# JonasGeiping/breaching

Hardware: NVIDIA H100
Metric: reconstruction iters/sec (ResNet-18 224x224, invertinggradients) (higher is better)
Workload: dtype tf32

## Files before the change

### breaching_b200/csrc/engine.cu

```cuda
#include <math.h>
#include <stdlib.h>
#include <string.h>

#include <limits>
#include <string>
#include <vector>

#include "../../include/breaching_b200.h"
#include "common.cuh"
#include "igemm.cuh"
#include "layers.cuh"
#include "tokens.cuh"
#include "objective.cuh"
#include "augment.cuh"

namespace bre {
void set_pdl(bool on);
static thread_local std::string g_last_error;
void set_error(const std::string& msg) { g_last_error = msg; }
static int g_pdl = -1;
bool use_pdl() {
  if (g_pdl < 0) {
    const char* e = getenv("BRE_PDL");
    g_pdl = e ? (atoi(e) != 0) : 1;
// ... 312 lines not shown
      a.x_sN = g.Ci; a.x_sP = g.Ci; a.x_sC = 1;
    } else {
      g.N = ti.N; g.H = ti.H; g.W = ti.W; g.Ci = ti.C; g.Ho = to.H; g.Wo = to.W; g.Co = to.C;
      g.R = op.R; g.S = op.S; g.stride = op.stride; g.pad = op.pad;
      if (op.tin == 0) { a.x_sN = (long long)ti.C * ti.H * ti.W; a.x_sP = 1; a.x_sC = ti.H * ti.W; }
      else { a.x_sN = (long long)ti.H * ti.W * ti.C; a.x_sP = ti.C; a.x_sC = 1; }
    }
    a.nsrc = 1;
    a.ws = ws; a.counters = gemm_counters; a.ws_tiles = ws_tiles; a.splits = 0;
    a.force_fp32 = is_precise(op_index(op)) ? 1 : 0;
    return a;
  }
  int gemm(const GemmArgs& a) { return gemm_on(a, stream); }
  bool weight_prefetch = [] { const char* e = getenv("BRE_TC_WPREFETCH"); return e ? atoi(e) != 0 : true; }();
  bool v_settled = false;
  bool inside(const float* p, const float* base, long long n) const { return base != nullptr && p >= base && p < base + n; }
  unsigned static_weights(const GemmArgs& a) const {
    if (!weight_prefetch || ms_steps > 0 || a.mode == GEMM_WGRAD) return 0u;
    unsigned mask = 0;
    for (int s = 0; s < a.nsrc; ++s) {
      const float* p = a.wgt[s];
      const bool model = inside(p, W, P_pad) || inside(p, Wt, P_pad) || (Wcol != nullptr && p == Wcol);
      const bool direction = v_settled && (inside(p, V, P_pad) || inside(p, Vt, P_pad));
      if (model || direction) mask |= 1u << s;
    }
    return mask;
  }
  int gemm_on(const GemmArgs& a, cudaStream_t st) {
    if (linear_tall_supported(a)) return launch_linear_tall(a, st);
    if (linear_small_preferred(a)) return launch_linear_small(a, st);
    if (gemm_backend == 1 && !a.force_fp32 && igemm_tc_supported(a)) {
      GemmArgs b = a;
      b.wgt_static = static_weights(a);
      return launch_igemm_tc(b, st);
    }
    return launch_igemm_simt(a, st);
  }

  bool fuses_with_next(size_t i, const GemmArgs& a) const {
    if (!fuse_bnact || gemm_backend != 1 || i + 1 >= ops.size()) return false;
    const bre_op_desc& nx = ops[i + 1];
    return nx.kind == BRE_OP_BNACT && nx.tin == ops[i].tout && !nx.bn_train && igemm_tc_supported(a);
  }
  std::vector<unsigned char> op_flags;
  void clear_op_flags(unsigned char bits) {
    op_flags.resize(ops.size(), 0);
    for (unsigned char& f : op_flags) f &= (unsigned char)~bits;
  }
  int consumers_of(int tensor) const {
    int n = 0;
    for (const bre_op_desc& o : ops) n += (o.tin == tensor) + (o.res == tensor);
    return n;
  }

  BnTrainArgs bn_train_args(const bre_op_desc& op) {
    const bre_tensor_desc& to = td(op.tout);
    const BnBuf& b = bn[op.bn_buffer];
    BnTrainArgs a;
    memset(&a, 0, sizeof(a));
    a.P = (long long)to.N * to.H * to.W; a.C = to.C; a.relu = op.relu != 0;
    a.in = t[op.tin].val; a.out = t[op.tout].val;
    a.inv = b.inv; a.nrm = b.nrm; a.scale = b.scale;
    a.v_gamma = Vp(op.gamma); a.v_beta = Vp(op.beta);
    a.sum_du = Gp(op.beta); a.sum_duxh = Gp(op.gamma);
    a.m1 = b.di_cm; a.m2 = b.di_cv; a.b1 = b.tb1; a.b2 = b.tb2;
    a.dout = t[op.tout].d; a.tdout = t[op.tout].td; a.xd = t[op.tin].tval;
// ... 1657 lines not shown
```

### breaching_b200/csrc/igemm.cuh

```cuda
#pragma once
#include "common.cuh"

namespace bre {

enum GemmMode { GEMM_FPROP = 0, GEMM_DGRAD = 1, GEMM_WGRAD = 2 };

struct ConvGeom {
  int N, H, W, Ci;
  int Ho, Wo, Co;
  int R, S, stride, pad;
};

struct GemmEpilogue {
  int kind;
  int has_bn, relu;
  int round_out;
  float* out2;
  const float* res;
  const float* scale;
  const float* shift;
  const float* inv;
  const float* nrm;
  const float* v_gamma;
  const float* v_beta;
  const float* pre;
  const float* post;
};

struct GemmArgs {
  int mode;
  GemmEpilogue epi;
  ConvGeom g;
  int nsrc;
  const float* act[2];
  const float* wgt[2];
  long long x_sN;
  int x_sP, x_sC;
  float* out;
  const float* bias;
  int accumulate;
  float* ws;
  int* counters;
  int ws_tiles;
  int splits;
  int force_fp32;
  unsigned wgt_static;
};

constexpr int IG_BM = 64, IG_BN = 64, IG_BK = 16, IG_THREADS = 256;

int launch_igemm_simt(const GemmArgs& a, cudaStream_t stream);
bool linear_small_supported(const GemmArgs& a);
int launch_linear_small(const GemmArgs& a, cudaStream_t stream);
bool linear_small_preferred(const GemmArgs& a);
bool linear_tall_supported(const GemmArgs& a);
int launch_linear_tall(const GemmArgs& a, cudaStream_t stream);
int launch_igemm_tc(const GemmArgs& a, cudaStream_t stream);
bool igemm_tc_supported(const GemmArgs& a);

inline void gemm_dims(const GemmArgs& a, int& M, int& Nc, int& K) {
  const ConvGeom& g = a.g;
  if (a.mode == GEMM_FPROP) { M = g.N * g.Ho * g.Wo; Nc = g.Co; K = g.R * g.S * g.Ci; }
  else if (a.mode == GEMM_DGRAD) { M = g.N * g.H * g.W; Nc = g.Ci; K = g.R * g.S * g.Co; }
  else { M = g.Co; Nc = g.R * g.S * g.Ci; K = g.N * g.Ho * g.Wo; }
}

}
```

### breaching_b200/csrc/igemm_tc.cu

```cuda
#include <stdlib.h>
#include <string.h>

#include <array>
#include <map>
#include <mutex>
#include <type_traits>

#include <cuda.h>

#include "igemm.cuh"

namespace bre {

namespace {

constexpr int TC_BM = 128;
constexpr int TC_BK = 32;
constexpr int TC_STAGES = 4;
constexpr int TC_MAX_STAGES = 8;
constexpr int TC_THREADS = 128;
constexpr int TC_BLOCK = 2 * TC_THREADS;

struct TcDims {
  int M, Nc, K;
// ... 138 lines not shown
               ::"r"(dst), "l"(reinterpret_cast<uint64_t>(tm)), "r"(smem_u32(bar)), "r"(c0), "r"(c1), "r"(c2) : "memory");
}

template <int NV>
__device__ __forceinline__ void fused_bnact(const GemmEpilogue& e, long long row, int n, float (&v)[NV]) {
  const long long o = row + n;
#pragma unroll
  for (int j = 0; j < NV; ++j) {
    float u = v[j];
    if (e.kind == 1) {
      if (e.has_bn) u = fmaf(u, __ldg(e.scale + n + j), __ldg(e.shift + n + j));
      if (e.res != nullptr) u += e.res[o + j];
      u = e.relu ? fmaxf(u, 0.f) : u;
      v[j] = e.round_out ? tf32_rna(u) : u;
    } else {
      if (e.has_bn) {
        const float xhat = fmaf(e.pre[o + j], __ldg(e.inv + n + j), __ldg(e.nrm + n + j));
        u = fmaf(__ldg(e.scale + n + j), u, fmaf(__ldg(e.v_gamma + n + j), xhat, __ldg(e.v_beta + n + j)));
      }
      if (e.res != nullptr) u += e.res[o + j];
      if (e.relu && !(e.post[o + j] > 0.f)) u = 0.f;
      v[j] = e.round_out ? tf32_rna(u) : u;
    }
  }
}

#ifdef BRE_TC_TRACE
__device__ long long g_tc_trace[16];
#define TC_MARK(i, cond) do { if ((cond) && blockIdx.x == 0 && blockIdx.y == 0 && blockIdx.z == 0) g_tc_trace[i] = clock64(); } while (0)
#else
#define TC_MARK(i, cond) do { } while (0)
#endif

template <int MODE, int BN, bool TMA, bool CLS = false>
__global__ void __launch_bounds__(TC_BLOCK) igemm_tc_kernel(GemmArgs a, TcDims d, int proxy_fence,
                                                            const __grid_constant__ std::conditional_t<CLS, TcMapsCls, TcMaps> maps, ClsPlan plan) {
  static_assert(!CLS || (MODE == GEMM_DGRAD && TMA), "per-class gathers: strided dgrad with the TMA producer only");
  constexpr uint32_t A_BYTES = TC_BM * TC_BK * 4, B_BYTES = BN * TC_BK * 4;
  extern __shared__ __align__(1024) uint8_t smem[];
  uint8_t* sA = smem;
  const int nst = 1 << d.stage_shift, stage_mask = nst - 1;
  uint8_t* sB = smem + nst * A_BYTES;
  __shared__ __align__(8) uint64_t bar_full[TC_MAX_STAGES];
  __shared__ __align__(8) uint64_t bar_empty[TC_MAX_STAGES];

  TC_MARK(0, threadIdx.x == 0);
  pdl_launch_dependents();
  const ConvGeom g = a.g;
  const int tid = threadIdx.x, warp = tid >> 5, lane = tid & 31;
  const int ptid = tid & (TC_THREADS - 1);
  const bool consumer = warp < TC_THREADS / 32;
  const int n0 = blockIdx.y * BN, z = blockIdx.z;
  int m0 = blockIdx.x * TC_BM;
  int kb_begin = z * d.kblocks_per_split;
  int kb_end = min(d.total_kblocks, kb_begin + d.kblocks_per_split);
  const int HoWo = g.Ho * g.Wo, HW = g.H * g.W;
  int cls = 0, cHc = 0, cWc = 0, cTy = 0, cTx = 0, cls_kps = 0, Mrows = d.M;
  if (CLS) {
#pragma unroll
    for (int c = 1; c < TC_MAXCLS; ++c)
      if (c < plan.ncls && (int)blockIdx.x >= plan.tile0[c]) cls = c;
    m0 = ((int)blockIdx.x - plan.tile0[cls]) * TC_BM;
    cHc = plan.Hc[cls]; cWc = plan.Wc[cls]; cTy = plan.Ty[cls]; cTx = plan.Tx[cls];
    Mrows = g.N * cHc * cWc;
    cls_kps = cTy * cTx * (g.Co / TC_BK);
    const int total = cls_kps * a.nsrc, per = (total + (int)gridDim.z - 1) / (int)gridDim.z;
    kb_begin = z * per;
    kb_end = min(total, kb_begin + per);
  }

  if (tid == 0) {
#pragma unroll
    for (int s = 0; s < TC_MAX_STAGES; ++s) { mbar_init(&bar_full[s], TMA ? 1 : TC_THREADS); mbar_init(&bar_empty[s], TC_THREADS / 32); }
    fence_barrier_init();
  }
  __syncthreads();
  TC_MARK(1, threadIdx.x == 0);

  constexpr bool a_mn = MODE == GEMM_WGRAD;
  constexpr bool b_mn = MODE != GEMM_FPROP;

  constexpr int A_VEC = TC_BM * TC_BK / 4 / TC_THREADS;
  constexpr int B_VEC = BN * TC_BK / 4 / TC_THREADS;
  const int gcol = ptid & 7, grow = (ptid >> 3) & 15;
  int a_off[A_VEC];
  unsigned long long a_taps[A_VEC];
  int a_yx[A_VEC];
  if (!TMA && !consumer && (MODE == GEMM_FPROP || MODE == GEMM_DGRAD)) {
#pragma unroll
    for (int j = 0; j < A_VEC; ++j) {
      const int m = m0 + grow + 16 * j;
      a_off[j] = 0; a_taps[j] = 0ull; a_yx[j] = 0;
      if (m < d.M) {
        if (MODE == GEMM_FPROP) {
          const int img = m / HoWo, rem = m - img * HoWo;
          const int p = rem / g.Wo, q = rem - p * g.Wo;
          const int y0 = p * g.stride - g.pad, x0 = q * g.stride - g.pad;
          a_off[j] = (int)(img * a.x_sN) + (y0 * g.W + x0) * a.x_sP + gcol * 4;
          for (int r = 0; r < g.R; ++r)
            for (int s2 = 0; s2 < g.S; ++s2)
              if (y0 + r >= 0 && y0 + r < g.H && x0 + s2 >= 0 && x0 + s2 < g.W) a_taps[j] |= 1ull << (r * g.S + s2);
        } else {
          const int img = m / HW, rem = m - img * HW;
          const int y = rem / g.W, x = rem - y * g.W;
          const int yb = y + g.pad, xb = x + g.pad;
          const int py = yb / g.stride, qx = xb / g.stride;
          const int ey = yb - py * g.stride, ex = xb - qx * g.stride;
          a_off[j] = ((img * g.Ho + py) * g.Wo + qx) * g.Co + gcol * 4;
          a_yx[j] = (ey << 16) | ex;
          for (int r = ey, pp = py; r < g.R; r += g.stride, --pp)
            for (int s2 = ex, qq = qx; s2 < g.S; s2 += g.stride, --qq)
              if (pp >= 0 && pp < g.Ho && qq >= 0 && qq < g.Wo) a_taps[j] |= 1ull << (r * g.S + s2);
        }
      }
    }
// ... 63 lines not shown
      return;
    }
    if (MODE == GEMM_WGRAD) {
      if (st.c0 >= d.kblocks_per_src * TC_BK) { st.c0 = 0; ++st.src; st.img = st.p = st.q = 0; }
      else {
        st.q += TC_BK;
        while (st.q >= g.Wo) { st.q -= g.Wo; if (++st.p == g.Ho) { st.p = 0; ++st.img; } }
      }
    } else if (st.c0 >= kch) {
      st.c0 = 0; ++st.rs;
      if (++st.s == g.S) { st.s = 0; if (++st.r == g.R) { st.r = 0; st.rs = 0; ++st.src; } }
    }
  };
  int wg_c[BN / 32], wg_r[BN / 32], wg_s[BN / 32];
  if (TMA && MODE == GEMM_WGRAD) {
#pragma unroll
    for (int h = 0; h < BN / 32; ++h) {
      const int n = n0 + 32 * h;
      const int rs = n / g.Ci;
      wg_c[h] = n - rs * g.Ci; wg_r[h] = rs / g.S; wg_s[h] = rs - wg_r[h] * g.S;
    }
  }
  auto issue_wgt_tma = [&](int stage, const KbState& st) {
    uint64_t* bar = &bar_full[stage];
    const uint32_t pb = smem_u32(sB) + stage * B_BYTES;
    if (MODE == GEMM_FPROP) {
      tma_tile2d(pb, &maps.wgt[st.src], bar, st.rs * g.Ci + st.c0, n0);
    } else if (MODE == GEMM_DGRAD) {
#pragma unroll
      for (int h = 0; h < BN / 32; ++h) tma_tile3d(pb + h * 4096, &maps.wgt[st.src], bar, n0 + 32 * h, st.rs, st.c0);
    } else {
      const uint32_t pa = smem_u32(sA) + stage * A_BYTES;
#pragma unroll
      for (int h = 0; h < TC_BM / 32; ++h) tma_tile2d(pa + h * 4096, &maps.wgt[st.src], bar, m0 + 32 * h, st.c0);
    }
  };
  auto issue_act_tma = [&](int stage, const KbState& st) {
    uint64_t* bar = &bar_full[stage];
    const uint32_t pa = smem_u32(sA) + stage * A_BYTES, pb = smem_u32(sB) + stage * B_BYTES;
    if (MODE == GEMM_FPROP) {
      tma_im2col(pa, &maps.act[st.src], bar, st.c0, base_w, base_h, base_n, st.s, st.r);
    } else if (MODE == GEMM_DGRAD) {
      if (CLS) tma_im2col(pa, &maps.act[2 * cls + st.src], bar, st.c0, base_w, base_h, base_n, cTx - 1 - st.s, cTy - 1 - st.r);
      else tma_im2col(pa, &maps.act[st.src], bar, st.c0, base_w, base_h, base_n, g.S - 1 - st.s, g.R - 1 - st.r);
    } else {
#pragma unroll
      for (int h = 0; h < BN / 32; ++h)
        tma_im2col(pb + h * 4096, &maps.act[st.src], bar, wg_c[h], st.q * g.stride - g.pad, st.p * g.stride - g.pad, st.img, wg_s[h], wg_r[h]);
    }
  };

  if (TMA && tid == 0 && (proxy_fence & 2)) {
    for (int sidx = 0; sidx < a.nsrc; ++sidx) {
      asm volatile("prefetch.tensormap [%0];" ::"l"(reinterpret_cast<uint64_t>(&maps.act[(CLS ? 2 * cls : 0) + sidx])) : "memory");
      asm volatile("prefetch.tensormap [%0];" ::"l"(reinterpret_cast<uint64_t>(&maps.wgt[sidx])) : "memory");
    }
  }
  const int nprod = (proxy_fence >> 2) & 7;
  const int pw = warp - TC_THREADS / 32;
  const bool producer = TMA && !consumer && lane == 0 && pw < nprod && pw < nkb;
  KbState pst;
  memset(&pst, 0, sizeof(pst));
  uint32_t pre_wgt = 0;
  if (producer) {
    pst = kb_init(kb_begin + pw);
    if (MODE != GEMM_WGRAD && a.wgt_static != 0) {
      KbState st = pst;
// ... 70 lines not shown
        }
      }
      {
        const int n4 = ptid & 15, kk = ptid >> 4;
        const int n = n0 + n4 * 4;
        const int rs = n / g.Ci, c = n - rs * g.Ci;
        const int r = rs / g.S, s = rs - r * g.S;
#pragma unroll
        for (int j = 0; j < B_VEC; ++j) {
          const int k = kk + 8 * j;
          const int pix = kbase + k;
          bool ok = pix < d.K;
          const float* gb = act;
          if (ok) {
            const int img = pix / HoWo, rem = pix - img * HoWo;
            const int p = rem / g.Wo, q = rem - p * g.Wo;
            const int h = p * g.stride - g.pad + r, w = q * g.stride - g.pad + s;
            ok = h >= 0 && h < g.H && w >= 0 && w < g.W;
            if (ok) gb = act + img * a.x_sN + (long long)(h * g.W + w) * a.x_sP + c;
          }
          cp_async16(pb + off_mn128(4 * n4, k), gb, ok ? 16u : 0u);
        }
      }
    }
    it_c0 += TC_BK;
    if (MODE == GEMM_WGRAD) {
      if (it_c0 >= d.kblocks_per_src * TC_BK) { it_c0 = 0; ++it_src; }
    } else if (it_c0 >= kch) {
      it_c0 = 0;
      if (++it_rs == g.R * g.S) { it_rs = 0; ++it_src; }
    }
  };

  float acc[2][BN / 2];
#pragma unroll
  for (int h = 0; h < 2; ++h)
#pragma unroll
    for (int i = 0; i < BN / 2; ++i) acc[h][i] = 0.f;
  const int gq = lane >> 2, tq = lane & 3;
  if (consumer) {
    for (int i = 0; i < nkb; ++i) {
      const int stage = i & stage_mask;
      mbar_wait(&bar_full[stage], (uint32_t)((i >> d.stage_shift) & 1));
      TC_MARK(4, i == 0 && tid == 0);
      if constexpr (MODE == GEMM_FPROP) {
        if (!TMA || (proxy_fence & 1)) fence_proxy_async();
        const uint32_t sa = smem_u32(sA) + stage * A_BYTES, sb = smem_u32(sB) + stage * B_BYTES;
        wgmma_fence();
#pragma unroll
        for (int j = 0; j < TC_BK / 8; ++j) {
          const uint64_t db = wgmma_desc_k128(sb + 32 * j);
          wgmma_tf32<BN>(acc[0], wgmma_desc_k128(sa + 32 * j), db);
          wgmma_tf32<BN>(acc[1], wgmma_desc_k128(sa + 64 * 128 + 32 * j), db);
        }
        wgmma_commit();
        wgmma_wait<1>();
        fence_regs(acc[0]);
        fence_regs(acc[1]);
        __syncwarp();
        if (i > 0 && lane == 0) mbar_arrive(&bar_empty[(i - 1) & stage_mask]);
      } else {
        const uint8_t* pa = sA + stage * A_BYTES;
        const uint8_t* pb = sB + stage * B_BYTES;
#pragma unroll
        for (int j = 0; j < TC_BK / 8; ++j) {
          const int k0 = 8 * j + tq;
          uint32_t af[2][4];
#pragma unroll
          for (int h = 0; h < 2; ++h) {
            const int r = 64 * h + 16 * warp + gq;
            af[h][0] = ld_op<a_mn>(pa, r, k0);
            af[h][1] = ld_op<a_mn>(pa, r + 8, k0);
            af[h][2] = ld_op<a_mn>(pa, r, k0 + 4);
            af[h][3] = ld_op<a_mn>(pa, r + 8, k0 + 4);
          }
#pragma unroll
          for (int jn = 0; jn < BN / 8; ++jn) {
            const uint32_t b0 = ld_op<b_mn>(pb, 8 * jn + gq, k0), b1 = ld_op<b_mn>(pb, 8 * jn + gq, k0 + 4);
            mma_tf32(&acc[0][4 * jn], af[0], b0, b1);
            mma_tf32(&acc[1][4 * jn], af[1], b0, b1);
          }
        }
        __syncwarp();
        if (lane == 0) mbar_arrive(&bar_empty[stage]);
      }
    }
    if constexpr (MODE == GEMM_FPROP) {
      wgmma_wait<0>();
      fence_regs(acc[0]);
      fence_regs(acc[1]);
    }
    TC_MARK(5, tid == 0);
  } else {
    if (TMA) {
      if (producer) {
        KbState st = pst;
        for (int i = pw; i < nkb; i += nprod) {
          const int stage = i & stage_mask;
          if (i >= nst) mbar_wait(&bar_empty[stage], (uint32_t)(((i >> d.stage_shift) - 1) & 1));
          if (i >= nst || !((pre_wgt >> i) & 1u)) {
            mbar_expect_tx(&bar_full[stage], A_BYTES + B_BYTES);
            issue_wgt_tma(stage, st);
          }
          issue_act_tma(stage, st);
          TC_MARK(3, i == (nkb < nst ? nkb : nst) - 1);
          for (int u = 0; u < nprod; ++u) kb_advance(st);
        }
      }
      __syncwarp();
    } else {
      for (int i = 0; i < nkb; ++i) {
        const int stage = i & stage_mask;
        if (i >= nst) mbar_wait(&bar_empty[stage], (uint32_t)(((i >> d.stage_shift) - 1) & 1));
        issue_block(stage);
        cp_async_arrive(&bar_full[stage]);
      }
      cp_async_wait<0>();
    }
  }

  const int splits = gridDim.z;
  auto out_row = [&](int mm, long long& row, int& cs) {
    if (CLS) {
      const int per = cHc * cWc;
      const int img = mm / per, rem = mm - img * per;
      const int iy = rem / cWc, ix = rem - iy * cWc;
      row = img * a.x_sN + (long long)((plan.y0[cls] + plan.stride * iy) * g.W + plan.x0[cls] + plan.stride * ix) * a.x_sP;
      cs = a.x_sC;
    } else if (MODE == GEMM_DGRAD) {
      const int img = mm / HW;
      row = img * a.x_sN + (long long)(mm - img * HW) * a.x_sP;
      cs = a.x_sC;
    } else {
      row = (long long)mm * d.Nc;
      cs = 1;
    }
  };
  if (consumer && splits == 1) {
#pragma unroll
    for (int h = 0; h < 2; ++h) {
#pragma unroll
      for (int hr = 0; hr < 2; ++hr) {
        const int mm = m0 + 64 * h + 16 * warp + gq + 8 * hr;
        if (mm >= Mrows) continue;
        long long row;
        int cs;
        out_row(mm, row, cs);
#pragma unroll
        for (int jn = 0; jn < BN / 8; ++jn) {
          const int n = n0 + 8 * jn + 2 * tq;
          float v[2] = {acc[h][4 * jn + 2 * hr], acc[h][4 * jn + 2 * hr + 1]};
          if (MODE == GEMM_FPROP && a.bias != nullptr) {
            v[0] += __ldg(a.bias + n);
            v[1] += __ldg(a.bias + n + 1);
          }
          float* op = a.out + row + (long long)n * cs;
          if (MODE == GEMM_FPROP && a.epi.kind != 0) {
            if (a.out != nullptr) *reinterpret_cast<float2*>(op) = make_float2(v[0], v[1]);
            fused_bnact<2>(a.epi, row, n, v);
            *reinterpret_cast<float2*>(a.epi.out2 + row + n) = make_float2(v[0], v[1]);
          } else if (cs == 1) {
            float2 t2 = make_float2(v[0], v[1]);
            if (a.accumulate) {
              const float2 o = *reinterpret_cast<const float2*>(op);
              t2.x += o.x; t2.y += o.y;
            }
            *reinterpret_cast<float2*>(op) = t2;
          } else {
#pragma unroll
            for (int j = 0; j < 2; ++j) {
              float* q = op + (long long)j * cs;
              *q = a.accumulate ? *q + v[j] : v[j];
            }
          }
        }
      }
    }
  } else if (consumer) {
    consumer_sync();
    float* part = reinterpret_cast<float*>(sA);
#pragma unroll
    for (int h = 0; h < 2; ++h) {
#pragma unroll
      for (int hr = 0; hr < 2; ++hr) {
        const int r = 64 * h + 16 * warp + gq + 8 * hr;
#pragma unroll
        for (int jn = 0; jn < BN / 8; ++jn) {
          const int c = 8 * jn + 2 * tq;
          const int chunk = (c >> 2) ^ (r & (BN / 4 - 1) & 15);
          *reinterpret_cast<float2*>(part + r * BN + chunk * 4 + (c & 3)) = make_float2(acc[h][4 * jn + 2 * hr], acc[h][4 * jn + 2 * hr + 1]);
        }
      }
    }
  }
  if (splits > 1) {
    TC_MARK(7, tid == 0);
    cluster_sync_all();
    TC_MARK(8, tid == 0);
    if (consumer) {
      auto reduce_rows = [&](auto s_tag) {
        constexpr int S = decltype(s_tag)::value;
        constexpr int C4 = BN / 4, SLOTS = (TC_BM / S) * C4 / TC_THREADS > 0 ? (TC_BM / S) * C4 / TC_THREADS : 1;
        const uint32_t part_s = smem_u32(sA);
        float4 t[SLOTS][S];
        int rr[SLOTS], cc[SLOTS];
#pragma unroll
        for (int sl = 0; sl < SLOTS; ++sl) {
          const int slot = tid + sl * TC_THREADS;
          rr[sl] = z * (TC_BM / S) + slot / C4;
          cc[sl] = slot % C4;
          const uint32_t local = part_s + (uint32_t)(rr[sl] * BN + ((cc[sl] ^ (rr[sl] & (BN / 4 - 1) & 15)) << 2)) * 4u;
#pragma unroll
          for (int q = 0; q < S; ++q) t[sl][q] = ld_dsmem4(local, (uint32_t)q);
        }
#pragma unroll
        for (int sl = 0; sl < SLOTS; ++sl) {
          const int r = rr[sl], c4 = cc[sl];
          if (m0 + r >= Mrows) continue;
          float4 acc4 = t[sl][0];
#pragma unroll
          for (int q = 1; q < S; ++q) { acc4.x += t[sl][q].x; acc4.y += t[sl][q].y; acc4.z += t[sl][q].z; acc4.w += t[sl][q].w; }
          const int n = n0 + c4 * 4;
          if (MODE == GEMM_FPROP && a.bias != nullptr) {
            acc4.x += __ldg(a.bias + n); acc4.y += __ldg(a.bias + n + 1); acc4.z += __ldg(a.bias + n + 2); acc4.w += __ldg(a.bias + n + 3);
          }
          long long row;
          int cs;
          out_row(m0 + r, row, cs);
          float* op = a.out + row + (long long)n * cs;
          if (MODE == GEMM_FPROP && a.epi.kind != 0) {
            if (a.out != nullptr) *reinterpret_cast<float4*>(op) = acc4;
            float vv[4] = {acc4.x, acc4.y, acc4.z, acc4.w};
            fused_bnact<4>(a.epi, row, n, vv);
            *reinterpret_cast<float4*>(a.epi.out2 + row + n) = make_float4(vv[0], vv[1], vv[2], vv[3]);
          } else if (cs == 1) {
            if (a.accumulate) {
              const float4 o = *reinterpret_cast<const float4*>(op);
              acc4.x += o.x; acc4.y += o.y; acc4.z += o.z; acc4.w += o.w;
            }
            *reinterpret_cast<float4*>(op) = acc4;
          } else {
            const float vv[4] = {acc4.x, acc4.y, acc4.z, acc4.w};
// ... 78 lines not shown

bool tiled_map(CUtensorMap* out, const float* base, int rank, const long long* dims_ll, const long long* strides_elems, const int* box_i,
               CUtensorMapSwizzle swz) {
  MapKey key = {1, (long long)reinterpret_cast<uintptr_t>(base), rank, (long long)swz};
  for (int i = 0; i < rank; ++i) { key[4 + i] = dims_ll[i]; key[8 + i] = box_i[i]; if (i + 1 < rank) key[12 + i] = strides_elems[i]; }
  std::lock_guard<std::mutex> lock(g_map_mutex);
  auto it = g_map_cache.find(key);
  if (it != g_map_cache.end()) { *out = it->second; return true; }
  const TmaApi& api = tma_api();
  if (!api.ok) return false;
  cuuint64_t dims[3], strides[2];
  cuuint32_t box[3], estr[3] = {1, 1, 1};
  for (int i = 0; i < rank; ++i) { dims[i] = (cuuint64_t)dims_ll[i]; box[i] = (cuuint32_t)box_i[i]; }
  for (int i = 0; i + 1 < rank; ++i) strides[i] = (cuuint64_t)strides_elems[i] * 4;
  CUtensorMap tm;
  const CUresult res = api.tiled(&tm, CU_TENSOR_MAP_DATA_TYPE_FLOAT32, (cuuint32_t)rank, const_cast<float*>(base), dims, strides, box, estr,
                                 CU_TENSOR_MAP_INTERLEAVE_NONE, swz, CU_TENSOR_MAP_L2_PROMOTION_L2_128B, CU_TENSOR_MAP_FLOAT_OOB_FILL_NONE);
  if (res != CUDA_SUCCESS) return false;
  g_map_cache.emplace(key, tm);
  *out = tm;
  return true;
}

bool tma_eligible(const GemmArgs& a) {
  static const int tma_env = [] { const char* e = getenv("BRE_TC_TMA"); return e ? atoi(e) : 1; }();
  if (!tma_env || !tma_api().ok) return false;
  const ConvGeom& g = a.g;
  if (g.stride > 8 || g.pad > 127 || g.R - 1 - g.pad > 127 || g.S - 1 - g.pad > 127 || g.R > 128 || g.S > 128) return false;
  if (a.mode == GEMM_DGRAD) return g.stride == 1;
  if (a.mode == GEMM_WGRAD) return g.Ci % 32 == 0;
  return true;
}

bool build_maps(const GemmArgs& a, int BN, TcMaps* maps) {
  const ConvGeom& g = a.g;
  const CUtensorMapSwizzle K128 = CU_TENSOR_MAP_SWIZZLE_128B;
  for (int s = 0; s < a.nsrc; ++s) {
    if (a.mode == GEMM_FPROP) {
      if (!im2col_map(&maps->act[s], a.act[s], g.N, g.H, g.W, g.Ci, a.x_sN, a.x_sP, -g.pad, -g.pad, g.pad - (g.S - 1), g.pad - (g.R - 1),
                      g.stride, TC_BK, TC_BM, K128))
        return false;
      const long long K = (long long)g.R * g.S * g.Ci;
      const long long dims[2] = {K, g.Co}, strides[1] = {K};
      const int box[2] = {TC_BK, BN};
      if (!tiled_map(&maps->wgt[s], a.wgt[s], 2, dims, strides, box, K128)) return false;
    } else if (a.mode == GEMM_DGRAD) {
      const int lw = g.pad - (g.S - 1), lh = g.pad - (g.R - 1);
      if (!im2col_map(&maps->act[s], a.act[s], g.N, g.Ho, g.Wo, g.Co, (long long)g.Ho * g.Wo * g.Co, g.Co, lw, lh, lw + g.W - g.Wo,
                      lh + g.H - g.Ho, 1, TC_BK, TC_BM, K128))
        return false;
      const long long dims[3] = {g.Ci, (long long)g.R * g.S, g.Co}, strides[2] = {g.Ci, (long long)g.R * g.S * g.Ci};
      const int box[3] = {32, 1, TC_BK};
      if (!tiled_map(&maps->wgt[s], a.wgt[s], 3, dims, strides, box, K128)) return false;
    } else {
      const long long npix = (long long)g.N * g.Ho * g.Wo;
      const long long dims[2] = {g.Co, npix}, strides[1] = {g.Co};
      const int box[2] = {32, TC_BK};
      if (!tiled_map(&maps->wgt[s], a.wgt[s], 2, dims, strides, box, K128)) return false;
      if (!im2col_map(&maps->act[s], a.act[s], g.N, g.H, g.W, g.Ci, a.x_sN, a.x_sP, -g.pad, -g.pad, g.pad - (g.S - 1), g.pad - (g.R - 1),
                      g.stride, 32, TC_BK, K128))
        return false;
    }
  }
  return true;
}

struct AxisPlan { bool any; int y0, Hc, T, L, U; };
inline AxisPlan axis_plan(int H, int Ho, int R, int stride, int pad, int e) {
  AxisPlan p{false, 0, 0, 0, 0, 0};
  p.y0 = ((e - pad) % stride + stride) % stride;
  if (p.y0 >= H) return p;
  p.any = true;
  p.Hc = (H - p.y0 + stride - 1) / stride;
  if (e >= R) return p;
  p.T = (R - e + stride - 1) / stride;
  const int c = (p.y0 + pad - e) / stride;
  p.L = c - (p.T - 1);
  p.U = p.Hc - Ho + p.L;
  return p;
}

bool cls_eligible(const GemmArgs& a) {
  static const int env = [] { const char* e = getenv("BRE_TC_STRIDED_TMA"); return e ? atoi(e) : 1; }();
  const ConvGeom& g = a.g;
  if (!env || a.mode != GEMM_DGRAD || g.stride != 2 || !tma_api().ok) return false;
  static const int tma_env = [] { const char* e = getenv("BRE_TC_TMA"); return e ? atoi(e) : 1; }();
  if (!tma_env || g.R > 16 || g.S > 16) return false;
  for (int ey = 0; ey < 2; ++ey)
    for (int horiz = 0; horiz < 2; ++horiz) {
      const AxisPlan p = horiz ? axis_plan(g.W, g.Wo, g.S, 2, g.pad, ey) : axis_plan(g.H, g.Ho, g.R, 2, g.pad, ey);
      if (p.any && p.T > 0 && (p.L < -128 || p.L > 127 || p.U < -128 || p.U > 127)) return false;
    }
  return true;
}

bool build_cls(const GemmArgs& a, ClsPlan* plan, TcMapsCls* maps) {
  const ConvGeom& g = a.g;
  memset(plan, 0, sizeof(*plan));
  plan->stride = g.stride;
  int tiles = 0, n = 0;
  for (int ey = 0; ey < g.stride; ++ey) {
    const AxisPlan py = axis_plan(g.H, g.Ho, g.R, g.stride, g.pad, ey);
    if (!py.any) continue;
    for (int ex = 0; ex < g.stride; ++ex) {
      const AxisPlan px = axis_plan(g.W, g.Wo, g.S, g.stride, g.pad, ex);
      if (!px.any) continue;
      if (n >= TC_MAXCLS) return false;
      const bool taps = py.T > 0 && px.T > 0;
      plan->Hc[n] = py.Hc; plan->Wc[n] = px.Hc; plan->y0[n] = py.y0; plan->x0[n] = px.y0;
      plan->Ty[n] = taps ? py.T : 0; plan->Tx[n] = taps ? px.T : 0;
      plan->Ly[n] = py.L; plan->Lx[n] = px.L; plan->ey[n] = ey; plan->ex[n] = ex;
      plan->tile0[n] = tiles;
      tiles += ceil_div((long long)g.N * py.Hc * px.Hc, TC_BM);
      for (int s = 0; s < a.nsrc && taps; ++s)
        if (!im2col_map(&maps->act[2 * n + s], a.act[s], g.N, g.Ho, g.Wo, g.Co, (long long)g.Ho * g.Wo * g.Co, g.Co, px.L, py.L, px.U, py.U, 1,
                        TC_BK, TC_BM, CU_TENSOR_MAP_SWIZZLE_128B))
          return false;
      if (!taps)
        for (int s = 0; s < a.nsrc; ++s) maps->act[2 * n + s] = maps->act[s];
      ++n;
    }
  }
  plan->ncls = n;
  plan->tile0[n] = tiles;
  for (int s = 0; s < a.nsrc; ++s) {
    const long long dims[3] = {g.Ci, (long long)g.R * g.S, g.Co}, strides[2] = {g.Ci, (long long)g.R * g.S * g.Ci};
    const int box[3] = {32, 1, TC_BK};
    if (!tiled_map(&maps->wgt[s], a.wgt[s], 3, dims, strides, box, CU_TENSOR_MAP_SWIZZLE_128B)) return false;
  }
  return n > 0;
}

template <int MODE, int BN, bool TMA, bool CLS = false>
int launch_tc(const GemmArgs& a, const TcDims& d0, const std::conditional_t<CLS, TcMapsCls, TcMaps>& maps, cudaStream_t stream,
              const ClsPlan* plan_in = nullptr) {
  TcDims d = d0;
  ClsPlan plan;
  memset(&plan, 0, sizeof(plan));
  if (CLS) plan = *plan_in;
  const int tm = CLS ? plan.tile0[plan.ncls] : ceil_div(d.M, TC_BM), tn = d.Nc / BN;
  if (CLS) {
    int kmax = 0;
    for (int c = 0; c < plan.ncls; ++c) kmax = kmax > plan.Ty[c] * plan.Tx[c] ? kmax : plan.Ty[c] * plan.Tx[c];
    d.total_kblocks = kmax * (a.g.Co / TC_BK) * a.nsrc;
    if (d.total_kblocks < 1) d.total_kblocks = 1;
  }
  const long long tiles = (long long)tm * tn;
  static const int max_splits_env = [] { const char* e = getenv("BRE_TC_MAX_SPLITS"); return e ? atoi(e) : 0; }();
  static const int target_ctas_env = [] { const char* e = getenv("BRE_TC_TARGET_CTAS"); return e ? atoi(e) : 0; }();
  const int target = target_ctas_env > 0 ? target_ctas_env : kNumSMs;
  constexpr int kMaxCluster = 8;
  int splits = a.splits;
  if (splits <= 0) {
    splits = 1;
    while (splits < kMaxCluster && tiles * splits < target && d.total_kblocks / (splits * 2) >= 2) splits *= 2;
  }
  if (max_splits_env > 0 && splits > max_splits_env) splits = max_splits_env;
  int pow2 = 1;
  while (pow2 * 2 <= splits && pow2 < kMaxCluster) pow2 *= 2;
  splits = pow2;
  while (splits > 1 && splits > d.total_kblocks) splits /= 2;
  d.kblocks_per_split = ceil_div(d.total_kblocks, splits);
  if (tn > 65535) { set_error("igemm_tc: grid too large"); return -1; }
  static const int stages_env = [] { const char* e = getenv("BRE_TC_STAGES"); return e ? atoi(e) : 0; }();
  static const int shortk_env = [] { const char* e = getenv("BRE_TC_SHORTK_STAGES"); return e ? atoi(e) : 2; }();
  const bool shortk = shortk_env == 2 && d.kblocks_per_split <= 6 && tm == 1 && tiles * splits > 2LL * kNumSMs;
  const int stages = (stages_env == 8 || stages_env == 2) ? stages_env : (shortk ? 2 : TC_STAGES);
  d.stage_shift = stages == 8 ? 3 : (stages == 2 ? 1 : 2);
  const size_t smem = (size_t)stages * (TC_BM + BN) * TC_BK * 4;
  const size_t smem_max = (size_t)TC_MAX_STAGES * (TC_BM + BN) * TC_BK * 4;
  static bool attr_done = false;
  if (!attr_done) {
    BRE_CUDA_CHECK(cudaFuncSetAttribute(igemm_tc_kernel<MODE, BN, TMA, CLS>, cudaFuncAttributeMaxDynamicSharedMemorySize, (int)smem_max));
    attr_done = true;
  }
  static const int proxy_fence_env = [] {
    const char* e = getenv("BRE_TC_PROXY_FENCE");
    const char* pf = getenv("BRE_TC_PREFETCH");
    const char* np = getenv("BRE_TC_PRODUCERS");
    int nprod = np ? atoi(np) : 2;
    if (nprod < 1 || nprod > 4) nprod = 2;
    return (e && atoi(e) ? 1 : 0) | ((pf ? atoi(pf) : 1) ? 2 : 0) | (nprod << 2);
  }();
  {
    cudaError_t lerr = launch_kernel(igemm_tc_kernel<MODE, BN, TMA, CLS>, dim3(tm, tn, splits), dim3(TC_BLOCK), smem, stream, splits, a, d,
                                     proxy_fence_env, maps, plan);
    if (lerr != cudaSuccess) { set_error(std::string("igemm_tc launch failed: ") + cudaGetErrorString(lerr)); return -2; }
  }
  BRE_CHECK_LAUNCH();
  return 0;
}

}

static bool narrow_tiles_ok(const GemmArgs& a) {
  static const int env = [] { const char* e = getenv("BRE_TC_NARROW"); return e ? atoi(e) : 1; }();
  if (!env || !tma_eligible(a)) return false;
  if (a.mode == GEMM_DGRAD && a.g.stride != 1) return false;
  if (a.mode == GEMM_WGRAD && (a.g.Ci % 32 != 0)) return false;
  return true;
}

bool igemm_tc_supported(const GemmArgs& a) {
  const ConvGeom& g = a.g;
  int M, Nc, K;
  gemm_dims(a, M, Nc, K);
  for (int s = 0; s < a.nsrc; ++s)
    if (!aligned16(a.act[s]) || !aligned16(a.wgt[s])) return false;
  if (!aligned16(a.out) || (a.splits == 0 && a.ws == nullptr)) return false;
  const bool x_nhwc = a.x_sC == 1 && a.x_sP % 4 == 0 && a.x_sN % 4 == 0;
  if (Nc % 64 != 0 && !(Nc % 32 == 0 && narrow_tiles_ok(a))) return false;
  switch (a.mode) {
    case GEMM_FPROP: return x_nhwc && g.Ci % TC_BK == 0 && g.R * g.S <= 64;
    case GEMM_DGRAD: return x_nhwc && g.Co % TC_BK == 0 && g.R * g.S <= 64;
    case GEMM_WGRAD: return x_nhwc && g.Co % 4 == 0 && g.Ci % 4 == 0 && g.R * g.S <= 64;
    default: return false;
  }
}

int launch_igemm_tc(const GemmArgs& a, cudaStream_t stream) {
  if (!igemm_tc_supported(a)) { set_error("igemm_tc: unsupported shape"); return -4; }
  TcDims d;
  gemm_dims(a, d.M, d.Nc, d.K);
  d.kblocks_per_src = ceil_div(d.K, TC_BK);
  d.total_kblocks = d.kblocks_per_src * a.nsrc;
  d.kblocks_per_split = d.total_kblocks;
  TcMaps maps;
  memset(&maps, 0, sizeof(maps));
  if (cls_eligible(a)) {
    ClsPlan plan;
    TcMapsCls cmaps;
    memset(&cmaps, 0, sizeof(cmaps));
    if (build_cls(a, &plan, &cmaps)) return launch_tc<GEMM_DGRAD, 64, true, true>(a, d, cmaps, stream, &plan);
  }
  const long long wide_tiles = (long long)ceil_div(d.M, TC_BM) * (d.Nc / 64);
  const bool underfilled = a.mode != GEMM_FPROP && d.Nc % 64 == 0 && wide_tiles * 16 <= kNumSMs && d.total_kblocks >= 64 &&
                           narrow_tiles_ok(a);
  if (d.Nc % 64 != 0 || (underfilled && build_maps(a, 32, &maps))) {
    if (d.Nc % 64 != 0 && !build_maps(a, 32, &maps)) { set_error("igemm_tc: tensor-map encoding failed for a narrow-tile shape"); return -4; }
    if (a.mode == GEMM_FPROP) return launch_tc<GEMM_FPROP, 32, true>(a, d, maps, stream);
    if (a.mode == GEMM_DGRAD) return launch_tc<GEMM_DGRAD, 32, true>(a, d, maps, stream);
    return launch_tc<GEMM_WGRAD, 32, true>(a, d, maps, stream);
  }
  const bool tma = tma_eligible(a) && build_maps(a, 64, &maps);
  if (a.mode == GEMM_FPROP) return tma ? launch_tc<GEMM_FPROP, 64, true>(a, d, maps, stream) : launch_tc<GEMM_FPROP, 64, false>(a, d, maps, stream);
  if (a.mode == GEMM_DGRAD) return tma ? launch_tc<GEMM_DGRAD, 64, true>(a, d, maps, stream) : launch_tc<GEMM_DGRAD, 64, false>(a, d, maps, stream);
  return tma ? launch_tc<GEMM_WGRAD, 64, true>(a, d, maps, stream) : launch_tc<GEMM_WGRAD, 64, false>(a, d, maps, stream);
}

}

#ifdef BRE_TC_TRACE
extern "C" int bre_debug_tc_trace(long long* out16) {
  return cudaMemcpyFromSymbol(out16, bre::g_tc_trace, sizeof(long long) * 16) == cudaSuccess ? 0 : -1;
}
#endif
```

Measured before the change: 672.5.

## Add 64-row tensor-core GEMM tiles for small-M fprop/dgrad convolutions

Templates the TC implicit-GEMM kernel on the M tile height and adds a 64-row variant for fprop/dgrad (including per-class strided dgrad) when the GEMM has at most 64 rows. Small-M layers stop computing and loading a half-empty 128-row tile, and the smaller tile fits a deeper 8-stage pipeline with a two-blocks-per-SM launch bound. The split-K plan is kept identical to the 128-row plan, with an error returned if it would differ, so results stay consistent. The variant is disabled in multi-step mode and can be toggled by an environment variable.

Result: faster. 713.0 (median of 6 runs) (+6.0%).

```diff
diff --git a/breaching_b200/csrc/engine.cu b/breaching_b200/csrc/engine.cu
--- a/breaching_b200/csrc/engine.cu
+++ b/breaching_b200/csrc/engine.cu
@@ -368,6 +368,7 @@
     if (gemm_backend == 1 && !a.force_fp32 && igemm_tc_supported(a)) {
       GemmArgs b = a;
       b.wgt_static = static_weights(a);
+      b.rows128 = ms_steps > 0 ? 1 : 0;
       return launch_igemm_tc(b, st);
     }
     return launch_igemm_simt(a, st);
diff --git a/breaching_b200/csrc/igemm.cuh b/breaching_b200/csrc/igemm.cuh
--- a/breaching_b200/csrc/igemm.cuh
+++ b/breaching_b200/csrc/igemm.cuh
@@ -45,6 +45,7 @@
   int splits;
   int force_fp32;
   unsigned wgt_static;
+  int rows128;
 };
 
 constexpr int IG_BM = 64, IG_BN = 64, IG_BK = 16, IG_THREADS = 256;
diff --git a/breaching_b200/csrc/igemm_tc.cu b/breaching_b200/csrc/igemm_tc.cu
--- a/breaching_b200/csrc/igemm_tc.cu
+++ b/breaching_b200/csrc/igemm_tc.cu
@@ -194,11 +194,13 @@
 #define TC_MARK(i, cond) do { } while (0)
 #endif
 
-template <int MODE, int BN, bool TMA, bool CLS = false>
-__global__ void __launch_bounds__(TC_BLOCK) igemm_tc_kernel(GemmArgs a, TcDims d, int proxy_fence,
+template <int MODE, int BN, bool TMA, bool CLS = false, int BM = TC_BM>
+__global__ void __launch_bounds__(TC_BLOCK, BM == TC_BM ? 0 : 2) igemm_tc_kernel(GemmArgs a, TcDims d, int proxy_fence,
                                                             const __grid_constant__ std::conditional_t<CLS, TcMapsCls, TcMaps> maps, ClsPlan plan) {
   static_assert(!CLS || (MODE == GEMM_DGRAD && TMA), "per-class gathers: strided dgrad with the TMA producer only");
-  constexpr uint32_t A_BYTES = TC_BM * TC_BK * 4, B_BYTES = BN * TC_BK * 4;
+  static_assert(BM == TC_BM || (BM == 64 && TMA && MODE != GEMM_WGRAD), "64-row tiles: fprop / dgrad with the TMA producer only");
+  constexpr int HM = BM / 64;
+  constexpr uint32_t A_BYTES = BM * TC_BK * 4, B_BYTES = BN * TC_BK * 4;
   extern __shared__ __align__(1024) uint8_t smem[];
   uint8_t* sA = smem;
   const int nst = 1 << d.stage_shift, stage_mask = nst - 1;
@@ -213,7 +215,7 @@
   const int ptid = tid & (TC_THREADS - 1);
   const bool consumer = warp < TC_THREADS / 32;
   const int n0 = blockIdx.y * BN, z = blockIdx.z;
-  int m0 = blockIdx.x * TC_BM;
+  int m0 = blockIdx.x * BM;
   int kb_begin = z * d.kblocks_per_split;
   int kb_end = min(d.total_kblocks, kb_begin + d.kblocks_per_split);
   const int HoWo = g.Ho * g.Wo, HW = g.H * g.W;
@@ -222,7 +224,7 @@
 #pragma unroll
     for (int c = 1; c < TC_MAXCLS; ++c)
       if (c < plan.ncls && (int)blockIdx.x >= plan.tile0[c]) cls = c;
-    m0 = ((int)blockIdx.x - plan.tile0[cls]) * TC_BM;
+    m0 = ((int)blockIdx.x - plan.tile0[cls]) * BM;
     cHc = plan.Hc[cls]; cWc = plan.Wc[cls]; cTy = plan.Ty[cls]; cTx = plan.Tx[cls];
     Mrows = g.N * cHc * cWc;
     cls_kps = cTy * cTx * (g.Co / TC_BK);
@@ -242,7 +244,7 @@
   constexpr bool a_mn = MODE == GEMM_WGRAD;
   constexpr bool b_mn = MODE != GEMM_FPROP;
 
-  constexpr int A_VEC = TC_BM * TC_BK / 4 / TC_THREADS;
+  constexpr int A_VEC = BM * TC_BK / 4 / TC_THREADS;
   constexpr int B_VEC = BN * TC_BK / 4 / TC_THREADS;
   const int gcol = ptid & 7, grow = (ptid >> 3) & 15;
   int a_off[A_VEC];
@@ -372,7 +374,7 @@
     } else {
       const uint32_t pa = smem_u32(sA) + stage * A_BYTES;
 #pragma unroll
-      for (int h = 0; h < TC_BM / 32; ++h) tma_tile2d(pa + h * 4096, &maps.wgt[st.src], bar, m0 + 32 * h, st.c0);
+      for (int h = 0; h < BM / 32; ++h) tma_tile2d(pa + h * 4096, &maps.wgt[st.src], bar, m0 + 32 * h, st.c0);
     }
   };
   auto issue_act_tma = [&](int stage, const KbState& st) {
@@ -509,9 +511,9 @@
     }
   };
 
-  float acc[2][BN / 2];
-#pragma unroll
-  for (int h = 0; h < 2; ++h)
+  float acc[HM][BN / 2];
+#pragma unroll
+  for (int h = 0; h < HM; ++h)
 #pragma unroll
     for (int i = 0; i < BN / 2; ++i) acc[h][i] = 0.f;
   const int gq = lane >> 2, tq = lane & 3;
@@ -527,13 +529,13 @@
 #pragma unroll
         for (int j = 0; j < TC_BK / 8; ++j) {
           const uint64_t db = wgmma_desc_k128(sb + 32 * j);
-          wgmma_tf32<BN>(acc[0], wgmma_desc_k128(sa + 32 * j), db);
-          wgmma_tf32<BN>(acc[1], wgmma_desc_k128(sa + 64 * 128 + 32 * j), db);
+#pragma unroll
+          for (int h = 0; h < HM; ++h) wgmma_tf32<BN>(acc[h], wgmma_desc_k128(sa + h * 64 * 128 + 32 * j), db);
         }
         wgmma_commit();
         wgmma_wait<1>();
-        fence_regs(acc[0]);
-        fence_regs(acc[1]);
+#pragma unroll
+        for (int h = 0; h < HM; ++h) fence_regs(acc[h]);
         __syncwarp();
         if (i > 0 && lane == 0) mbar_arrive(&bar_empty[(i - 1) & stage_mask]);
       } else {
@@ -542,9 +544,9 @@
 #pragma unroll
         for (int j = 0; j < TC_BK / 8; ++j) {
           const int k0 = 8 * j + tq;
-          uint32_t af[2][4];
-#pragma unroll
-          for (int h = 0; h < 2; ++h) {
+          uint32_t af[HM][4];
+#pragma unroll
+          for (int h = 0; h < HM; ++h) {
             const int r = 64 * h + 16 * warp + gq;
             af[h][0] = ld_op<a_mn>(pa, r, k0);
             af[h][1] = ld_op<a_mn>(pa, r + 8, k0);
@@ -554,8 +556,8 @@
 #pragma unroll
           for (int jn = 0; jn < BN / 8; ++jn) {
             const uint32_t b0 = ld_op<b_mn>(pb, 8 * jn + gq, k0), b1 = ld_op<b_mn>(pb, 8 * jn + gq, k0 + 4);
-            mma_tf32(&acc[0][4 * jn], af[0], b0, b1);
-            mma_tf32(&acc[1][4 * jn], af[1], b0, b1);
+#pragma unroll
+            for (int h = 0; h < HM; ++h) mma_tf32(&acc[h][4 * jn], af[h], b0, b1);
           }
         }
         __syncwarp();
@@ -564,8 +566,8 @@
     }
     if constexpr (MODE == GEMM_FPROP) {
       wgmma_wait<0>();
-      fence_regs(acc[0]);
-      fence_regs(acc[1]);
+#pragma unroll
+      for (int h = 0; h < HM; ++h) fence_regs(acc[h]);
     }
     TC_MARK(5, tid == 0);
   } else {
@@ -615,7 +617,7 @@
   };
   if (consumer && splits == 1) {
 #pragma unroll
-    for (int h = 0; h < 2; ++h) {
+    for (int h = 0; h < HM; ++h) {
 #pragma unroll
       for (int hr = 0; hr < 2; ++hr) {
         const int mm = m0 + 64 * h + 16 * warp + gq + 8 * hr;
@@ -657,7 +659,7 @@
     consumer_sync();
     float* part = reinterpret_cast<float*>(sA);
 #pragma unroll
-    for (int h = 0; h < 2; ++h) {
+    for (int h = 0; h < HM; ++h) {
 #pragma unroll
       for (int hr = 0; hr < 2; ++hr) {
         const int r = 64 * h + 16 * warp + gq + 8 * hr;
@@ -677,14 +679,15 @@
     if (consumer) {
       auto reduce_rows = [&](auto s_tag) {
         constexpr int S = decltype(s_tag)::value;
-        constexpr int C4 = BN / 4, SLOTS = (TC_BM / S) * C4 / TC_THREADS > 0 ? (TC_BM / S) * C4 / TC_THREADS : 1;
+        constexpr int C4 = BN / 4, NSLOT = (BM / S) * C4, SLOTS = NSLOT / TC_THREADS > 0 ? NSLOT / TC_THREADS : 1;
         const uint32_t part_s = smem_u32(sA);
         float4 t[SLOTS][S];
         int rr[SLOTS], cc[SLOTS];
+        if (NSLOT < TC_THREADS && tid >= NSLOT) return;
 #pragma unroll
         for (int sl = 0; sl < SLOTS; ++sl) {
           const int slot = tid + sl * TC_THREADS;
-          rr[sl] = z * (TC_BM / S) + slot / C4;
+          rr[sl] = z * (BM / S) + slot / C4;
           cc[sl] = slot % C4;
           const uint32_t local = part_s + (uint32_t)(rr[sl] * BN + ((cc[sl] ^ (rr[sl] & (BN / 4 - 1) & 15)) << 2)) * 4u;
 #pragma unroll
@@ -829,13 +832,13 @@
   return true;
 }
 
-bool build_maps(const GemmArgs& a, int BN, TcMaps* maps) {
+bool build_maps(const GemmArgs& a, int BN, int BM, TcMaps* maps) {
   const ConvGeom& g = a.g;
   const CUtensorMapSwizzle K128 = CU_TENSOR_MAP_SWIZZLE_128B;
   for (int s = 0; s < a.nsrc; ++s) {
     if (a.mode == GEMM_FPROP) {
       if (!im2col_map(&maps->act[s], a.act[s], g.N, g.H, g.W, g.Ci, a.x_sN, a.x_sP, -g.pad, -g.pad, g.pad - (g.S - 1), g.pad - (g.R - 1),
-                      g.stride, TC_BK, TC_BM, K128))
+                      g.stride, TC_BK, BM, K128))
         return false;
       const long long K = (long long)g.R * g.S * g.Ci;
       const long long dims[2] = {K, g.Co}, strides[1] = {K};
@@ -844,7 +847,7 @@
     } else if (a.mode == GEMM_DGRAD) {
       const int lw = g.pad - (g.S - 1), lh = g.pad - (g.R - 1);
       if (!im2col_map(&maps->act[s], a.act[s], g.N, g.Ho, g.Wo, g.Co, (long long)g.Ho * g.Wo * g.Co, g.Co, lw, lh, lw + g.W - g.Wo,
-                      lh + g.H - g.Ho, 1, TC_BK, TC_BM, K128))
+                      lh + g.H - g.Ho, 1, TC_BK, BM, K128))
         return false;
       const long long dims[3] = {g.Ci, (long long)g.R * g.S, g.Co}, strides[2] = {g.Ci, (long long)g.R * g.S * g.Ci};
       const int box[3] = {32, 1, TC_BK};
@@ -891,7 +894,18 @@
   return true;
 }
 
-bool build_cls(const GemmArgs& a, ClsPlan* plan, TcMapsCls* maps) {
+long long cls_rows_max(const GemmArgs& a) {
+  const ConvGeom& g = a.g;
+  long long rows = 0;
+  for (int ey = 0; ey < g.stride; ++ey)
+    for (int ex = 0; ex < g.stride; ++ex) {
+      const AxisPlan py = axis_plan(g.H, g.Ho, g.R, g.stride, g.pad, ey), px = axis_plan(g.W, g.Wo, g.S, g.stride, g.pad, ex);
+      if (py.any && px.any && (long long)g.N * py.Hc * px.Hc > rows) rows = (long long)g.N * py.Hc * px.Hc;
+    }
+  return rows;
+}
+
+bool build_cls(const GemmArgs& a, int BM, ClsPlan* plan, TcMapsCls* maps) {
   const ConvGeom& g = a.g;
   memset(plan, 0, sizeof(*plan));
   plan->stride = g.stride;
@@ -908,10 +922,10 @@
       plan->Ty[n] = taps ? py.T : 0; plan->Tx[n] = taps ? px.T : 0;
       plan->Ly[n] = py.L; plan->Lx[n] = px.L; plan->ey[n] = ey; plan->ex[n] = ex;
       plan->tile0[n] = tiles;
-      tiles += ceil_div((long long)g.N * py.Hc * px.Hc, TC_BM);
+      tiles += ceil_div((long long)g.N * py.Hc * px.Hc, BM);
       for (int s = 0; s < a.nsrc && taps; ++s)
         if (!im2col_map(&maps->act[2 * n + s], a.act[s], g.N, g.Ho, g.Wo, g.Co, (long long)g.Ho * g.Wo * g.Co, g.Co, px.L, py.L, px.U, py.U, 1,
-                        TC_BK, TC_BM, CU_TENSOR_MAP_SWIZZLE_128B))
+                        TC_BK, BM, CU_TENSOR_MAP_SWIZZLE_128B))
           return false;
       if (!taps)
         for (int s = 0; s < a.nsrc; ++s) maps->act[2 * n + s] = maps->act[s];
@@ -928,21 +942,7 @@
   return n > 0;
 }
 
-template <int MODE, int BN, bool TMA, bool CLS = false>
-int launch_tc(const GemmArgs& a, const TcDims& d0, const std::conditional_t<CLS, TcMapsCls, TcMaps>& maps, cudaStream_t stream,
-              const ClsPlan* plan_in = nullptr) {
-  TcDims d = d0;
-  ClsPlan plan;
-  memset(&plan, 0, sizeof(plan));
-  if (CLS) plan = *plan_in;
-  const int tm = CLS ? plan.tile0[plan.ncls] : ceil_div(d.M, TC_BM), tn = d.Nc / BN;
-  if (CLS) {
-    int kmax = 0;
-    for (int c = 0; c < plan.ncls; ++c) kmax = kmax > plan.Ty[c] * plan.Tx[c] ? kmax : plan.Ty[c] * plan.Tx[c];
-    d.total_kblocks = kmax * (a.g.Co / TC_BK) * a.nsrc;
-    if (d.total_kblocks < 1) d.total_kblocks = 1;
-  }
-  const long long tiles = (long long)tm * tn;
+int split_factor(const GemmArgs& a, long long tiles, int total_kblocks) {
   static const int max_splits_env = [] { const char* e = getenv("BRE_TC_MAX_SPLITS"); return e ? atoi(e) : 0; }();
   static const int target_ctas_env = [] { const char* e = getenv("BRE_TC_TARGET_CTAS"); return e ? atoi(e) : 0; }();
   const int target = target_ctas_env > 0 ? target_ctas_env : kNumSMs;
@@ -950,25 +950,56 @@
   int splits = a.splits;
   if (splits <= 0) {
     splits = 1;
-    while (splits < kMaxCluster && tiles * splits < target && d.total_kblocks / (splits * 2) >= 2) splits *= 2;
+    while (splits < kMaxCluster && tiles * splits < target && total_kblocks / (splits * 2) >= 2) splits *= 2;
   }
   if (max_splits_env > 0 && splits > max_splits_env) splits = max_splits_env;
   int pow2 = 1;
   while (pow2 * 2 <= splits && pow2 < kMaxCluster) pow2 *= 2;
   splits = pow2;
-  while (splits > 1 && splits > d.total_kblocks) splits /= 2;
+  while (splits > 1 && splits > total_kblocks) splits /= 2;
+  return splits;
+}
+
+template <int MODE, int BN, bool TMA, bool CLS = false, int BM = TC_BM>
+int launch_tc(const GemmArgs& a, const TcDims& d0, const std::conditional_t<CLS, TcMapsCls, TcMaps>& maps, cudaStream_t stream,
+              const ClsPlan* plan_in = nullptr) {
+  TcDims d = d0;
+  ClsPlan plan;
+  memset(&plan, 0, sizeof(plan));
+  if (CLS) plan = *plan_in;
+  const int tm = CLS ? plan.tile0[plan.ncls] : ceil_div(d.M, BM), tn = d.Nc / BN;
+  long long tm128 = CLS ? 0 : ceil_div(d.M, TC_BM);
+  if (CLS) {
+    int kmax = 0;
+    for (int c = 0; c < plan.ncls; ++c) {
+      kmax = kmax > plan.Ty[c] * plan.Tx[c] ? kmax : plan.Ty[c] * plan.Tx[c];
+      tm128 += ceil_div((long long)a.g.N * plan.Hc[c] * plan.Wc[c], TC_BM);
+    }
+    d.total_kblocks = kmax * (a.g.Co / TC_BK) * a.nsrc;
+    if (d.total_kblocks < 1) d.total_kblocks = 1;
+  }
+  const int splits = split_factor(a, tm128 * tn, d.total_kblocks);
   d.kblocks_per_split = ceil_div(d.total_kblocks, splits);
+  if (BM != TC_BM) {
+    const int own = split_factor(a, (long long)tm * tn, d.total_kblocks);
+    if (own != splits || ceil_div(d.total_kblocks, own) != d.kblocks_per_split) {
+      set_error("igemm_tc: 64-row tiles would change the split-K plan of the 128-row tiles");
+      return -4;
+    }
+  }
   if (tn > 65535) { set_error("igemm_tc: grid too large"); return -1; }
   static const int stages_env = [] { const char* e = getenv("BRE_TC_STAGES"); return e ? atoi(e) : 0; }();
   static const int shortk_env = [] { const char* e = getenv("BRE_TC_SHORTK_STAGES"); return e ? atoi(e) : 2; }();
+  const long long tiles = (long long)tm * tn;
   const bool shortk = shortk_env == 2 && d.kblocks_per_split <= 6 && tm == 1 && tiles * splits > 2LL * kNumSMs;
-  const int stages = (stages_env == 8 || stages_env == 2) ? stages_env : (shortk ? 2 : TC_STAGES);
+  constexpr bool deep = (size_t)TC_MAX_STAGES * (BM + BN) * TC_BK * 4 <= (size_t)TC_STAGES * (TC_BM + 64) * TC_BK * 4;
+  const int stages = (stages_env == 8 || stages_env == 4 || stages_env == 2) ? stages_env : (shortk ? 2 : (deep ? TC_MAX_STAGES : TC_STAGES));
   d.stage_shift = stages == 8 ? 3 : (stages == 2 ? 1 : 2);
-  const size_t smem = (size_t)stages * (TC_BM + BN) * TC_BK * 4;
-  const size_t smem_max = (size_t)TC_MAX_STAGES * (TC_BM + BN) * TC_BK * 4;
+  const size_t smem = (size_t)stages * (BM + BN) * TC_BK * 4;
+  const size_t smem_max = (size_t)TC_MAX_STAGES * (BM + BN) * TC_BK * 4;
   static bool attr_done = false;
   if (!attr_done) {
-    BRE_CUDA_CHECK(cudaFuncSetAttribute(igemm_tc_kernel<MODE, BN, TMA, CLS>, cudaFuncAttributeMaxDynamicSharedMemorySize, (int)smem_max));
+    BRE_CUDA_CHECK(cudaFuncSetAttribute(igemm_tc_kernel<MODE, BN, TMA, CLS, BM>, cudaFuncAttributeMaxDynamicSharedMemorySize, (int)smem_max));
     attr_done = true;
   }
   static const int proxy_fence_env = [] {
@@ -980,7 +1011,7 @@
     return (e && atoi(e) ? 1 : 0) | ((pf ? atoi(pf) : 1) ? 2 : 0) | (nprod << 2);
   }();
   {
-    cudaError_t lerr = launch_kernel(igemm_tc_kernel<MODE, BN, TMA, CLS>, dim3(tm, tn, splits), dim3(TC_BLOCK), smem, stream, splits, a, d,
+    cudaError_t lerr = launch_kernel(igemm_tc_kernel<MODE, BN, TMA, CLS, BM>, dim3(tm, tn, splits), dim3(TC_BLOCK), smem, stream, splits, a, d,
                                      proxy_fence_env, maps, plan);
     if (lerr != cudaSuccess) { set_error(std::string("igemm_tc launch failed: ") + cudaGetErrorString(lerr)); return -2; }
   }
@@ -1024,22 +1055,36 @@
   d.kblocks_per_split = d.total_kblocks;
   TcMaps maps;
   memset(&maps, 0, sizeof(maps));
+  static const int bm64_env = [] { const char* e = getenv("BRE_TC_BM64"); return e ? atoi(e) : 1; }();
+  const bool bm64_ok = bm64_env && !a.rows128;
   if (cls_eligible(a)) {
     ClsPlan plan;
     TcMapsCls cmaps;
     memset(&cmaps, 0, sizeof(cmaps));
-    if (build_cls(a, &plan, &cmaps)) return launch_tc<GEMM_DGRAD, 64, true, true>(a, d, cmaps, stream, &plan);
-  }
+    if (bm64_ok && cls_rows_max(a) <= 64) {
+      if (build_cls(a, 64, &plan, &cmaps)) return launch_tc<GEMM_DGRAD, 64, true, true, 64>(a, d, cmaps, stream, &plan);
+    } else if (build_cls(a, TC_BM, &plan, &cmaps)) {
+      return launch_tc<GEMM_DGRAD, 64, true, true>(a, d, cmaps, stream, &plan);
+    }
+  }
+  const bool rows64 = bm64_ok && d.M <= 64 && a.mode != GEMM_WGRAD && tma_eligible(a);
+  const int bm = rows64 ? 64 : TC_BM;
   const long long wide_tiles = (long long)ceil_div(d.M, TC_BM) * (d.Nc / 64);
   const bool underfilled = a.mode != GEMM_FPROP && d.Nc % 64 == 0 && wide_tiles * 16 <= kNumSMs && d.total_kblocks >= 64 &&
                            narrow_tiles_ok(a);
-  if (d.Nc % 64 != 0 || (underfilled && build_maps(a, 32, &maps))) {
-    if (d.Nc % 64 != 0 && !build_maps(a, 32, &maps)) { set_error("igemm_tc: tensor-map encoding failed for a narrow-tile shape"); return -4; }
-    if (a.mode == GEMM_FPROP) return launch_tc<GEMM_FPROP, 32, true>(a, d, maps, stream);
-    if (a.mode == GEMM_DGRAD) return launch_tc<GEMM_DGRAD, 32, true>(a, d, maps, stream);
+  if (d.Nc % 64 != 0 || (underfilled && build_maps(a, 32, bm, &maps))) {
+    if (d.Nc % 64 != 0 && !build_maps(a, 32, bm, &maps)) { set_error("igemm_tc: tensor-map encoding failed for a narrow-tile shape"); return -4; }
+    if (a.mode == GEMM_FPROP)
+      return rows64 ? launch_tc<GEMM_FPROP, 32, true, false, 64>(a, d, maps, stream) : launch_tc<GEMM_FPROP, 32, true>(a, d, maps, stream);
+    if (a.mode == GEMM_DGRAD)
+      return rows64 ? launch_tc<GEMM_DGRAD, 32, true, false, 64>(a, d, maps, stream) : launch_tc<GEMM_DGRAD, 32, true>(a, d, maps, stream);
     return launch_tc<GEMM_WGRAD, 32, true>(a, d, maps, stream);
   }
-  const bool tma = tma_eligible(a) && build_maps(a, 64, &maps);
+  const bool tma = tma_eligible(a) && build_maps(a, 64, bm, &maps);
+  if (tma && rows64) {
+    if (a.mode == GEMM_FPROP) return launch_tc<GEMM_FPROP, 64, true, false, 64>(a, d, maps, stream);
+    return launch_tc<GEMM_DGRAD, 64, true, false, 64>(a, d, maps, stream);
+  }
   if (a.mode == GEMM_FPROP) return tma ? launch_tc<GEMM_FPROP, 64, true>(a, d, maps, stream) : launch_tc<GEMM_FPROP, 64, false>(a, d, maps, stream);
   if (a.mode == GEMM_DGRAD) return tma ? launch_tc<GEMM_DGRAD, 64, true>(a, d, maps, stream) : launch_tc<GEMM_DGRAD, 64, false>(a, d, maps, stream);
   return tma ? launch_tc<GEMM_WGRAD, 64, true>(a, d, maps, stream) : launch_tc<GEMM_WGRAD, 64, false>(a, d, maps, stream);
```
